# igashov/DiffLinker

Hardware: AMD Instinct MI355X
Metric: molecules/sec (500-step sample_chain) (higher is better)
Workload: dtype f32 (f16x3 split MFMA, fp32 accumulate)

## Files before the change

difflinker_amd/csrc/egnn_fc.hip:

```cpp
#include <hip/hip_runtime.h>
#include <stdint.h>
#include <stdlib.h>
#include <string.h>
#include <math.h>
#include <cmath>

#include <algorithm>
#include <atomic>
#include <vector>

#include "../../include/difflinker_hip.h"
#include "pack_layout.h"
#include "slot_order.h"


namespace {

constexpr int LDH = 132;
constexpr int NMAX = 55;
constexpr int NQMAX = 2 * NMAX;
constexpr int THREADS = 512;
constexpr int NWAVES = THREADS / 64;
constexpr int GWAVES = 8;
constexpr int GTHREADS = 64 * GWAVES;
constexpr int L_A = 0;
constexpr int L_B = L_A + NMAX * LDH;
constexpr int L_C = L_B + NMAX * LDH;
constexpr int L_W = L_C + NMAX * LDH;
constexpr int L_VEC = L_W + UNIT;
constexpr int L_XS = L_VEC + 4 * HID;
constexpr int L_X0 = L_XS + NQMAX * 4;
constexpr int L_Z = L_X0 + NQMAX * 4;
constexpr int L_LM = L_Z + NMAX * DMAX;
constexpr int L_FRAG = L_LM + 56;
constexpr int L_IDX = L_FRAG + 56;
constexpr int L_RCV = L_IDX + 112;
constexpr int L_RPOS = L_RCV + 56;
constexpr int L_MISC = L_RPOS + 56;
constexpr int MISC_WORDS = 40;
constexpr int L_FMAX = L_MISC + MISC_WORDS;
constexpr int L_DUMMY = L_FMAX + 8;
constexpr int L_PROG = L_DUMMY + LDH;
constexpr int L_TOTAL = L_PROG + 8;
constexpr int L_ZROW = L_XS + 4 * 56;
static_assert(L_ZROW + HID <= L_X0 && 56 >= NMAX + 1 && (L_ZROW % 4) == 0, "the zero row sits in the team-only part of the coordinate rows");
constexpr size_t LDS_BYTES = size_t(L_TOTAL) * 4;
static_assert(LDS_BYTES <= 163840, "LDS layout exceeds 160 KiB");
static_assert((L_B % 4) == 0 && (L_C % 4) == 0 && (L_W % 4) == 0 && (L_VEC % 4) == 0 && (L_XS % 4) == 0 &&
              (L_X0 % 4) == 0 && (L_Z % 4) == 0 && (L_DUMMY % 4) == 0, "16-byte alignment");
constexpr int L_TRIP3 = L_A + 2 * ST_CHUNK;
constexpr int L_AGGX3 = L_TRIP3 + 4 * 256;
static_assert(L_AGGX3 + 4 * (NMAX + 1) <= L_W && (L_TRIP3 % 4) == 0, "version-3 coordinate scratch must fit the h region behind the ring");

constexpr int TM_EPOCH = 2;
constexpr int TM_FAIL = 3;
constexpr int TM_ROWS = 4;
constexpr int TM_FLAGS = 6;
constexpr int TM_S = 8, TM_RANK = 9, TM_NOWN = 10;
constexpr int MS_NRCV = 12;
constexpr int MS_FULL = 13;
constexpr int CX_V3 = 38;

struct Lds {
    float *A, *B, *C, *W, *vec, *xs, *x0, *aggx, *z, *lm, *frag;
    int *idx, *rcv, *rpos, *misc;
    unsigned* fmax;
    float* dummy;
    int w;
};

__device__ __forceinline__ Lds lds_view(float* base) {
    Lds v;
    v.w = __builtin_amdgcn_readfirstlane(int(threadIdx.x) >> 6);
    v.A = base + L_A; v.B = base + L_B; v.C = base + L_C; v.W = base + L_W; v.vec = base + L_VEC;
    v.xs = base + L_XS; v.x0 = base + L_X0; v.z = base + L_Z;
    v.aggx = base + L_B;
    v.lm = base + L_LM; v.frag = base + L_FRAG;
    v.idx = reinterpret_cast<int*>(base + L_IDX); v.misc = reinterpret_cast<int*>(base + L_MISC);
    v.rcv = reinterpret_cast<int*>(base + L_RCV); v.rpos = reinterpret_cast<int*>(base + L_RPOS);
    v.fmax = reinterpret_cast<unsigned*>(base + L_FMAX);
    v.dummy = base + L_DUMMY;
    return v;
}

constexpr int PROF_MAX_EVENTS = 1024;
struct Prof {
    unsigned long long* buf;
    int n;
};
__device__ __forceinline__ void prof_event(Prof& pf, int w, int lane, int tag) {
#ifdef DL_PROFILE
    if (pf.buf != nullptr) {
        if (lane == 0 && pf.n < PROF_MAX_EVENTS) {
            unsigned long long* e = pf.buf + (size_t(w) * PROF_MAX_EVENTS + pf.n) * 2;
            e[0] = (unsigned long long)tag;
            e[1] = __builtin_amdgcn_s_memtime();
        }
        pf.n++;
    }
#else
    (void)pf; (void)w; (void)lane; (void)tag;
#endif
}

__device__ __forceinline__ void fine_event(Prof& pf, int w, int lane, int tag) {
// ... 68 lines not shown
    q.tid = 64 * q.w + q.lane;
    asm volatile("" : "+v"(q.tid));
    q.c = q.lane & 31; q.hh = q.lane >> 5;
    q.nt = q.w & 3; q.mt = q.w >> 2;
    return q;
}
struct NextPass {
    const float* base;
    bool equiv;
};
__device__ __forceinline__ void stage_next(const Lds& v, const NextPass& nx, int w, int tid) {
    if (nx.base == nullptr) return;
    stage_dma(v, nx.base + (nx.equiv ? E_W6T : G_W2T), nx.base + (nx.equiv ? E_VEC : G_VEC) + HID,
              nx.base + (nx.equiv ? E_VEC + 4 * HID : G_VEC + 6 * HID), w, tid);
}

__device__ __forceinline__ void store_row(const Lds& v, float* buf, int row, int nb, int col, float val) {
    float* p = (row < nb) ? buf + row * LDH + col : v.dummy + col;
    *p = val;
}

constexpr int FM_H0 = 0, FM_H1 = 1, FM_HG = 2, FM_AGG = 3, FM_XOWN = 4, FM_X2 = 5, FM_X02 = 6;

template <bool TEAM>
__device__ __forceinline__ float geo_scale(const Lds& v, const float* __restrict__ sc) {
    const float x2 = __uint_as_float(v.fmax[FM_X2]), x02 = __uint_as_float(v.fmax[FM_X02]);
    return fminf(scale_for(4.0f * x2) * scale_for(sc[6]), scale_for(4.0f * x02) * scale_for(sc[7]));
}

static_assert(SLOT_WAVES == GWAVES, "slot_order.h plans for the workgroup's waves");
constexpr int PB_STRIDE = LDH;
static_assert(NSLOT * PB_STRIDE <= L_W + UNIT, "partial-sum buffer must fit the P, Q, H, W2' regions");

#ifdef DL_TEST_HOOKS
__device__ int g_slots_receiver_major = 0;
#endif

__device__ __forceinline__ void split8t(const float (&u)[8], uint4& hi, uint4& lo) {
    unsigned h[4], l[4];
#pragma unroll
    for (int q = 0; q < 4; ++q) {
        const float a = u[2 * q], b = u[2 * q + 1];
        const float ah = __uint_as_float(__float_as_uint(a) & 0xffffe000u), bh = __uint_as_float(__float_as_uint(b) & 0xffffe000u);
        h[q] = __builtin_bit_cast(unsigned, __builtin_amdgcn_cvt_pkrtz(ah, bh));
        l[q] = __builtin_bit_cast(unsigned, __builtin_amdgcn_cvt_pkrtz(a - ah, b - bh));
    }
    hi = make_uint4(h[0], h[1], h[2], h[3]);
    lo = make_uint4(l[0], l[1], l[2], l[3]);
}

template <bool EQUIV, int PREC, bool ATT, bool TEAM>
__device__ __forceinline__ void pair_phase(const Lds& v, int nb, int w, int lane, const int8_t* __restrict__ emask, int N,
                                           float norm_constant, float sa, float inv_scale, const float* __restrict__ sc,
                                           float head, Prof& pf) {
    const int c = lane & 31, hh = lane >> 5;
    const int nrec = EQUIV ? v.misc[MS_NRCV] : (TEAM ? v.misc[TM_NOWN] : nb);
    const int S = TEAM ? v.misc[TM_S] : 1, rank = TEAM ? v.misc[TM_RANK] : 0;
#ifdef DL_TEST_HOOKS
    const SlotOrder so = slot_order(nrec, nb, g_slots_receiver_major != 0);
#else
    const SlotOrder so = slot_order(nrec, nb);
#endif
    const SlotLane sl = slot_lane(so, nb, 32 * w + c);
    const int q = so.q;
    const int nt = slot_wave_steps(so, w);
    const bool slot_ok = sl.ok;
    const int il = sl.il;
    const int li = EQUIV ? (slot_ok ? v.rcv[il] : 0) : il;
    const int i = rank + li * S;
    const int j0 = sl.j0;
    const int jn = sl.jn;
    const bool wave_active = nt > 0;

    floatx16 agg[4];
    float ax = 0.0f, ay = 0.0f, az = 0.0f;
#pragma unroll
    for (int mt = 0; mt < 4; ++mt) agg[mt] = splat16(0.0f);

    if (wave_active) {
        const float4 xi = *reinterpret_cast<const float4*>(v.xs + 4 * i);
        const float4 yi = *reinterpret_cast<const float4*>(v.x0 + 4 * i);
        const int8_t* mrow = emask ? emask + v.idx[i] * N : nullptr;
        const float* Pp_ = v.A + li * LDH + 4 * hh;
        const float* bias_p_ = v.vec + 2 * HID + 4 * hh;
        const float* w7_p_ = v.vec + 3 * HID + 4 * hh;
        float isa_s[8];
#pragma unroll
        for (int s_ = 0; s_ < 8; ++s_)
            isa_s[s_] = (PREC == 0) ? 1.0f
                : __int_as_float(__builtin_amdgcn_readfirstlane(__float_as_int(inv_pow2(sa * cload(sc, (EQUIV ? ES_NE : GS_NE) + s_)))));

        float ga[4];
        uint4 gaf[4];
        float sX = 1.0f, invS1 = 1.0f;
        if constexpr (PREC == 0) {
#pragma unroll
            for (int mt = 0; mt < 4; ++mt) ga[mt] = v.vec[(hh ? HID : 0) + 32 * mt + c];
        } else {
            const float s_wr = scale_for(sc[6]), s_wd = scale_for(sc[7]);
            const float S1 = geo_scale<TEAM>(v, sc);
            invS1 = inv_pow2(S1);
            sX = S1 * inv_pow2(hh ? s_wd : s_wr);
            const float s_w = hh ? s_wd : s_wr;
#pragma unroll
            for (int mt = 0; mt < 4; ++mt) {
                const float wv = v.vec[(hh ? HID : 0) + 32 * mt + c] * s_w;
                const float wh = __uint_as_float(__float_as_uint(wv) & 0xffffe000u);
// ... 241 lines not shown
                            __builtin_amdgcn_sched_barrier(0);
                        }
                    }
                } else
#pragma unroll
                for (int s = 0; s < 8; ++s) {
#pragma unroll
                    for (int i = 0; i < 12; ++i) {
                        const int m6 = i % 6, ge = 4 * (s + 1) + i / 3, ph = i % 3;
                        if (m6 == 0) {
                            const int ng = 2 * s + i / 6 + 1;
                            if (ng < 16) load_a(ng >> 1, ng & 1);
                        }
                        mfma_i(s, i);
                        if (i < 4 && s < 6 && !(s & 1)) load_qc((s + 2) >> 1, i);
                        if (i == 10 && s < 6 && !(s & 1)) g1 = mfma_h(gaf[(s + 2) >> 1], xf, Qc);
                        if (s < 7) {
                            if (ph == 0) { if ((ge & 1) == 0 && (ge >> 1) + 1 < 16) load_pq((ge >> 1) + 1); chunk_a(ge); }
                            if (ph == 1) chunk_b(ge);
                            if (ph == 2) chunk_c(ge);
                        }
                        __builtin_amdgcn_sched_barrier(0);
                    }
                }
                loop_event(pf, w, lane, 52);
                const float m = ok ? float(m_raw) : 0.0f;
                TileVecs tv[2];
                tv[0] = load_vecs(0);
#pragma unroll
                for (int mt = 0; mt < 4; ++mt) {
                    keep_vecs(tv[mt & 1]);
                    if (mt < 3) tv[(mt + 1) & 1] = load_vecs(mt + 1);
                    __builtin_amdgcn_sched_barrier(0);
                    epilogue(c2[mt], mt, tv[mt & 1], m);
                }
                if (ATT) attend(c2, m);
                loop_event(pf, w, lane, 53);
            }
            if (EQUIV) {
                float lo, hi;
                both_halves(ssum, lo, hi);
                float s_all = lo + hi;
                if (head != 0.0f)
                    s_all = head * (1.0f - 2.0f * __builtin_amdgcn_rcpf(1.0f + __builtin_amdgcn_exp2f(2.8853900817779268f * s_all)));
                const float den = sqrtf(r + 1e-8f) + norm_constant;
                const float f = ok ? s_all * float(m_raw) : 0.0f;
                ax += (dx / den) * f; ay += (dy / den) * f; az += (dz / den) * f;
            }
        }
        if (nt < q && lane == 0) prog[w] = q;
    }
    __builtin_amdgcn_s_setprio(0);
    prof_event(pf, w, lane, EQUIV ? 121 : 120);
    lds_barrier();
    if (lane == 0) reinterpret_cast<int*>(v.A - L_A + L_PROG)[w] = 0;
    int slot_w = 32 * w + c;
    asm volatile("" : "+v"(slot_w));
    const SlotLane sw = slot_lane(so, nb, slot_w);
    const int prow = sw.il * so.g + sw.c;
    float* pb = v.A + prow * PB_STRIDE;
    if (sw.ok) {
        if (!EQUIV) {
#pragma unroll
            for (int mt = 0; mt < 4; ++mt)
#pragma unroll
                for (int qq = 0; qq < 4; ++qq)
                    *reinterpret_cast<float4*>(pb + 32 * mt + 8 * qq + 4 * hh) =
                        make_float4(agg[mt][4 * qq], agg[mt][4 * qq + 1], agg[mt][4 * qq + 2], agg[mt][4 * qq + 3]);
        } else if (hh == 0) {
            *reinterpret_cast<float4*>(v.A + (v.misc[CX_V3] != 0 ? L_TRIP3 - L_A : 0) + 4 * prow) = make_float4(ax, ay, az, 0.0f);
        }
    }
}

struct AggRegs {
    float4 v[4];
};
__device__ __forceinline__ float pair_reduce_gcl(const Lds& v, int nown, int nb, int tid, AggRegs& out, float scale) {
    const SlotPlan pl = slot_plan(nown, nb);
    float am = 0.0f;
    const float* src[4];
    float4 s[4];
#pragma unroll
    for (int k = 0; k < 4; ++k) {
        const int e = tid + THREADS * k;
        src[k] = v.A + max(min(e >> 5, nown - 1), 0) * pl.g * PB_STRIDE + 4 * (e & 31);
        s[k] = make_float4(0.f, 0.f, 0.f, 0.f);
    }
    int ch = 0;
    for (; ch + 4 <= pl.g; ch += 4) {
        float4 p[4][4];
#pragma unroll
        for (int u = 0; u < 4; ++u)
#pragma unroll
            for (int k = 0; k < 4; ++k) p[u][k] = *reinterpret_cast<const float4*>(src[k] + (ch + u) * PB_STRIDE);
#pragma unroll
        for (int u = 0; u < 4; ++u)
#pragma unroll
            for (int k = 0; k < 4; ++k) { s[k].x += p[u][k].x; s[k].y += p[u][k].y; s[k].z += p[u][k].z; s[k].w += p[u][k].w; }
    }
    for (; ch < pl.g; ++ch) {
        float4 p[4];
#pragma unroll
        for (int k = 0; k < 4; ++k) p[k] = *reinterpret_cast<const float4*>(src[k] + ch * PB_STRIDE);
#pragma unroll
        for (int k = 0; k < 4; ++k) { s[k].x += p[k].x; s[k].y += p[k].y; s[k].z += p[k].z; s[k].w += p[k].w; }
// ... 556 lines not shown
    const int S = TEAM ? ctx_i(v, TM_S) : 1, rank = TEAM ? ctx_i(v, TM_RANK) : 0;
    float* hs = cx.hs;
    const NextPass nx = cx.nx;
    const LaneIds q = lane_ids(v);
    const int tid = q.tid, w = q.w, lane = q.lane;
    PreW2 pw;
    load_pre2(pw, nx, w, lane, nown);
    __builtin_amdgcn_sched_barrier(0);
    lds_barrier();
    const float xscale = (cx.flags & 4) ? 1.0f / float(N) : ((cx.flags & 2) ? ctx_f(v, CX_INVNORM) : 1.0f);
    pair_reduce_equiv<false>(v, nown, nb, tid, xscale);
    if (TEAM && tid == 0) v.fmax[FM_XOWN] = 0u;
    lds_barrier();
    stage_next(v, nx, w, tid);
    if constexpr (TEAM) {
        if (nb > NMAX && nx.base != nullptr)
            for (int e = tid; e < nown * 32; e += THREADS)
                *reinterpret_cast<float4*>(v.C + (e >> 5) * LDH + 4 * (e & 31)) = *reinterpret_cast<const float4*>(hs + HS_HF + (e >> 5) * HID + 4 * (e & 31));
    } else {
        if (tid == 0) v.fmax[FM_X2] = 0u;
        lds_barrier();
    }
    float n2 = 0.0f;
    if (tid < nown) {
        const float lm = v.lm[tid];
        const int a = rank + tid * S;
        const bool moves = v.rpos[tid] >= 0;
#pragma unroll
        for (int k = 0; k < 3; ++k) {
            float xn = v.xs[4 * a + k];
            if (moves) {
                xn += v.aggx[4 * tid + k] * lm;
                v.xs[4 * a + k] = xn;
            }
            n2 = fmaf(xn, xn, n2);
        }
    }
    block_max(&v.fmax[TEAM ? FM_XOWN : FM_X2], n2, lane);
    prof_event(pf, w, lane, 34);
    lds_barrier();
    prof_event(pf, w, lane, 10);
    open_pass<PREC, TEAM>(v, nb, nown, nx, hs, pf, pw, cx.pass + 1, cx.par);
}


typedef float floatx4 __attribute__((ext_vector_type(4)));
__device__ __forceinline__ floatx4 mfma16(const uint4& a, const uint4& b, floatx4 c) {
    return __builtin_amdgcn_mfma_f32_16x16x32_f16(__builtin_bit_cast(half8, a), __builtin_bit_cast(half8, b), c, 0, 0, 0);
}
constexpr int ST_AWAVES = 4;
constexpr int ST_PIECES = ST_CHUNK / 256 / 4;
__host__ __device__ constexpr int st_slot_off(int slot) { return slot < 2 ? L_W + slot * ST_CHUNK : L_A + (slot - 2) * ST_CHUNK; }
static_assert(L_A + 2 * ST_CHUNK <= L_W && 2 * ST_CHUNK == UNIT, "ring slots 2, 3 must fit below the W2' region");
__host__ __device__ constexpr int st_slot(int c, int nc) { return (c + ((4 - nc) & 3)) & 3; }

struct BOp {
    uint4 hi[4], lo[4];
};
__device__ __forceinline__ float4* st_tile(float* tiles, int w, int ot, int lane) {
    return reinterpret_cast<float4*>(tiles) + (w * 8 + ot) * 64 + lane;
}
__device__ __forceinline__ void st_load_rows(BOp& b, const float* rows, int l, int kg, float s) {
    const float* rp = rows + l * LDH + 4 * kg;
#pragma unroll
    for (int sl = 0; sl < 4; ++sl) {
        const float4 a = *reinterpret_cast<const float4*>(rp + 32 * sl), c4 = *reinterpret_cast<const float4*>(rp + 32 * sl + 16);
        const float u[8] = {a.x * s, a.y * s, a.z * s, a.w * s, c4.x * s, c4.y * s, c4.z * s, c4.w * s};
        split8t(u, b.hi[sl], b.lo[sl]);
    }
}
template <int SLOT>
__device__ __forceinline__ void st_mma_chunk(const float* lds0, const BOp& b, floatx4 (&acc)[4], int lane) {
    const uint4* Wc = reinterpret_cast<const uint4*>(lds0 + st_slot_off(SLOT)) + lane;
#pragma unroll
    for (int t = 0; t < 4; ++t) acc[t] = floatx4{0.f, 0.f, 0.f, 0.f};
#pragma unroll
    for (int sl = 0; sl < 4; ++sl) {
        uint4 ah[4], al[4];
#ifdef DL_KO_DSR
#pragma unroll
        for (int t = 0; t < 4; ++t) { ah[t] = b.hi[(sl + t) & 3]; al[t] = b.lo[(sl + t) & 3]; }
#else
#pragma unroll
        for (int t = 0; t < 4; ++t) { ah[t] = Wc[((t * 4 + sl) * 2 + 0) * 64]; al[t] = Wc[((t * 4 + sl) * 2 + 1) * 64]; }
#endif
#ifdef DL_KO_MFMA
#pragma unroll
        for (int t = 0; t < 4; ++t) { acc[t][0] += __uint_as_float(al[t].x ^ ah[t].y); acc[t][1] += __uint_as_float(al[t].z ^ ah[t].w); }
#else
#pragma unroll
        for (int t = 0; t < 4; ++t) acc[t] = mfma16(al[t], b.hi[sl], acc[t]);
#pragma unroll
        for (int t = 0; t < 4; ++t) acc[t] = mfma16(ah[t], b.lo[sl], acc[t]);
#pragma unroll
        for (int t = 0; t < 4; ++t) acc[t] = mfma16(ah[t], b.hi[sl], acc[t]);
#endif
    }
}
template <int SLOT>
__device__ __forceinline__ void st_issue(float* lds0, const float* __restrict__ src, int hw, int lane) {
    typedef const __attribute__((address_space(1))) void* gptr_t;
    typedef __attribute__((address_space(3))) void* lptr_t;
    const float4* s4 = reinterpret_cast<const float4*>(src) + lane;
#ifdef DL_KO_DMA
    (void)s4; (void)lds0; (void)hw;
#else
#pragma unroll
    for (int it = 0; it < ST_PIECES; ++it) {
        const int piece = it * 4 + hw;
        __builtin_amdgcn_global_load_lds((gptr_t)(s4 + piece * 64), (lptr_t)(lds0 + st_slot_off(SLOT) + piece * 256), 16, 0, 0);
    }
#endif
}
template <int HALF>
__device__ __forceinline__ void st_issue_image(const Lds& v, const NextPass& nx, int hw, int lane) {
    typedef const __attribute__((address_space(1))) void* gptr_t;
    typedef __attribute__((address_space(3))) void* lptr_t;
    const float* wimg = nx.base + (nx.equiv ? E_W6T : G_W2T);
    const float* vecs = nx.base + (nx.equiv ? E_VEC : G_VEC) + HID;
    const float* vec4 = nx.base + (nx.equiv ? E_VEC + 4 * HID : G_VEC + 6 * HID);
    if (HALF == 1 && hw < 2) {
        const int t2 = 64 * hw + lane;
        const float4* src = (t2 < 96) ? reinterpret_cast<const float4*>(vecs) + t2 : reinterpret_cast<const float4*>(vec4) + (t2 - 96);
        __builtin_amdgcn_global_load_lds((gptr_t)src, (lptr_t)(v.vec + 256 * hw), 16, 0, 0);
    }
    const float4* s4 = reinterpret_cast<const float4*>(wimg) + lane;
#pragma unroll
    for (int it = 0; it < ST_PIECES; ++it) {
        const int piece = HALF * 32 + it * 4 + hw;
        __builtin_amdgcn_global_load_lds((gptr_t)(s4 + piece * 64), (lptr_t)(v.W + piece * 256), 16, 0, 0);
    }
}
template <int N>
__device__ __forceinline__ void st_wait_vm() {
    if constexpr (N <= 0) asm volatile("s_waitcnt vmcnt(0)" ::: "memory");
    else asm volatile("s_waitcnt vmcnt(%0)" :: "n"(N) : "memory");
}
template <int V>
struct IC { static constexpr int value = V; };

template <bool TEAM, bool POST, bool NEXT_EQ>
__device__ __forceinline__ void stream_phase(const Lds& v, Prof& pf, const AggRegs* ar) {
    constexpr int NC = (POST ? 6 : 0) + 4;
    constexpr int C_P = POST ? 6 : 0;
    const PassCtx cx = pass_ctx(v);
    const LaneIds q = lane_ids(v);
    const int tid = q.tid, w = q.w, lane = q.lane;
    const int nb = cx.nb;
    const int nown = TEAM ? ctx_i(v, TM_NOWN) : nb;
    float* hs = cx.hs;
    const int pass_open = cx.pass + 1;
    const float* wp = ctx_p<const float>(v, CX_WP);
    const int sub = ctx_i(v, CX_SUB);
    const float* g = POST ? cx.g : nullptr;
    const float* nxb = pass_weights(wp, pass_open, sub);
    const NextPass nx = {nxb, NEXT_EQ};
    const float* sc = POST ? g + G_SCALE : nullptr;
    const float* scn = nxb + (NEXT_EQ ? E_SCALE : G_SCALE);
    const float* vecn = nxb + (NEXT_EQ ? E_VEC : G_VEC);
    float* lds0 = v.A - L_A;
    const bool loader = w >= ST_AWAVES;
    const int hw = w - ST_AWAVES, wa = w;
    const int n = lane & 15, kg = lane >> 4;
    const int ta = wa;
    const int l = 16 * ta + n;
    const bool awave = !loader && 16 * ta < nown;
    const bool valid = awave && l < nown;
    const int lc = max(min(l, nown - 1), 0);
    auto chunk_src = [&](int c) -> const float* {
        if (POST && c < C_P) return g + G_ST_POST + c * ST_CHUNK;
        return nxb + (NEXT_EQ ? E_ST_PRE : G_ST_PRE) + (c - C_P) * ST_CHUNK;
    };
    float4 hold[8];
    if (awave) {
#pragma unroll
        for (int ot = 0; ot < 8; ++ot) hold[ot] = *st_tile(hs + HS_HT, ta, ot, lane);
    }
    const int par = cx.par;
    float hmax = 0.f, aggmax = 0.f, s_agg = 1.f, s_t = 1.f, s_hn = 1.f, inv2 = 1.f;
    if constexpr (POST) {
        hmax = __uint_as_float(v.fmax[FM_H0 + par]);
        aggmax = __uint_as_float(v.fmax[FM_AGG]);
        s_agg = scale_for(aggmax);
        const float y3b = cload(sc, SC_L1_W3A) * hmax + cload(sc, SC_L1_W3B) * aggmax + cload(sc, SC_B3);
        s_t = scale_for(y3b);
        const float hnb = hmax + cload(sc, SC_L1_W4) * y3b + cload(sc, SC_B4);
        s_hn = scale_for(hnb);
        if (tid == 0 && (beyond_f16_range(aggmax) || beyond_f16_range(y3b) || beyond_f16_range(hnb))) atomicOr(&v.misc[1], NAN_RANGE | 3);
        inv2 = inv_pow2(s_t * cload(sc, 4));
    }
    const float s_h0 = scale_for(__uint_as_float(v.fmax[FM_H0 + par]));
    const float s_hf = POST ? s_hn : s_h0;
    constexpr int AGG_OFF = st_slot_off(st_slot(3, NC));
    if constexpr (POST) {
#pragma unroll
        for (int k = 0; k < 4; ++k) {
            const int e = tid + THREADS * k;
            if (e < nown * 32) *reinterpret_cast<float4*>(lds0 + AGG_OFF + (e >> 5) * LDH + 4 * (e & 31)) = ar->v[k];
        }
    }
    if (loader) {
        st_issue<st_slot(0, NC)>(lds0, chunk_src(0), hw, lane);
        prof_event(pf, w, lane, 200);
        auto lstep = [&](auto C_) {
            constexpr int C = decltype(C_)::value;
            constexpr int behind = (C >= 1 && C + 1 < NC ? ST_PIECES : 0) + (C == NC - 2 ? ST_PIECES : 0) + (C == NC - 1 ? 2 * ST_PIECES : 0);
            st_wait_vm<behind>();
            fine_event(pf, w, lane, 220 + C);
            lds_barrier();
            fine_event(pf, w, lane, 210 + C);
            if constexpr (C == 0) {
                st_issue<st_slot(1, NC)>(lds0, chunk_src(1), hw, lane);
                st_issue<st_slot(2, NC)>(lds0, chunk_src(2), hw, lane);
            }
            if constexpr (C == 1) st_wait_vm<ST_PIECES>();
            if constexpr (C >= 1 && C + 2 < NC) st_issue<st_slot(C + 2, NC)>(lds0, chunk_src(C + 2), hw, lane);
            if constexpr (C == NC - 3) st_issue_image<0>(v, nx, hw, lane);
            if constexpr (C == NC - 2) st_issue_image<1>(v, nx, hw, lane);
        };
        lstep(IC<0>{}); lstep(IC<1>{}); lstep(IC<2>{}); lstep(IC<3>{});
        if constexpr (NC > 4) { lstep(IC<4>{}); lstep(IC<5>{}); }
        if constexpr (NC > 6) { lstep(IC<6>{}); lstep(IC<7>{}); }
        if constexpr (NC > 8) { lstep(IC<8>{}); lstep(IC<9>{}); }
        fine_event(pf, w, lane, 240);
        lds_barrier();
        prof_event(pf, w, lane, 250);
    } else {
    BOp bh, bagg, bout, bin;
    floatx4 acc[4];
    float4 t0p[4];
    float4 res2[8], bb4[8];
    float4 Pout[8], Qout[8];
    float hm = 0.f;
    float S1 = 1.f;
    if (!TEAM) {
        const float x2 = __uint_as_float(v.fmax[FM_X2]), x02 = __uint_as_float(v.fmax[FM_X02]);
        S1 = fminf(scale_for(4.0f * x2) * scale_for(cload(scn, 6)), scale_for(4.0f * x02) * scale_for(cload(scn, 7)));
    }
    const float live = valid ? 1.0f : 0.0f;
    if (awave) {
        const float sb = s_h0 * live;
#pragma unroll
        for (int sl = 0; sl < 4; ++sl) {
            const float4 a = hold[2 * sl], c4 = hold[2 * sl + 1];
            const float u[8] = {a.x * sb, a.y * sb, a.z * sb, a.w * sb, c4.x * sb, c4.y * sb, c4.z * sb, c4.w * sb};
            split8t(u, bh.hi[sl], bh.lo[sl]);
        }
    }
    prof_event(pf, w, lane, 200);
    auto step = [&](auto C_) {
        constexpr int C = decltype(C_)::value;
        fine_event(pf, w, lane, 230 + C);
        lds_barrier();
        fine_event(pf, w, lane, 210 + C);
        if (!awave) return;
        constexpr bool IS_T0 = POST && C < 4 && (C & 1) == 0, IS_MLP1 = POST && C < 4 && (C & 1) == 1, IS_MLP2 = POST && (C == 4 || C == 5);
        constexpr bool IS_P = C >= C_P && C < C_P + 2;
        constexpr int half = (POST && C < 4) ? (C >> 1) : (C & 1);
        float4 bias[4];
        if constexpr (IS_P || IS_T0) {
#pragma unroll
            for (int t = 0; t < 4; ++t)
                bias[t] = *reinterpret_cast<const float4*>((IS_T0 ? g + G_VEC + 4 * HID : vecn) + 16 * (4 * half + t) + 4 * kg);
        }
        if constexpr (POST && C == 3) {
#pragma unroll
            for (int ot = 0; ot < 8; ++ot) {
                res2[ot] = *st_tile(hs + HS_HT, ta, ot, lane);
                bb4[ot] = *reinterpret_cast<const float4*>(g + G_VEC + 5 * HID + 16 * ot + 4 * kg);
            }
        }
        if constexpr (POST && C == 0) st_load_rows(bagg, lds0 + AGG_OFF, lc, kg, s_agg * live);
        if constexpr (IS_T0) st_mma_chunk<st_slot(C, NC)>(lds0, bh, acc, lane);
        else if constexpr (IS_MLP1) st_mma_chunk<st_slot(C, NC)>(lds0, bagg, acc, lane);
        else if constexpr (IS_MLP2) st_mma_chunk<st_slot(C, NC)>(lds0, bin, acc, lane);
        else st_mma_chunk<st_slot(C, NC)>(lds0, POST ? bin : bh, acc, lane);
        float4 res[4];
#pragma unroll
        for (int t = 0; t < 4; ++t) {
            const int ot = 4 * half + t, nt = ot >> 1;
            if constexpr (IS_T0) {
                const float inv = inv_pow2(s_h0 * cload(sc, GS_SW_W3A + nt));
                const float4 b3 = bias[t];
                t0p[t] = make_float4(fmaf(acc[t][0], inv, b3.x), fmaf(acc[t][1], inv, b3.y), fmaf(acc[t][2], inv, b3.z), fmaf(acc[t][3], inv, b3.w));
            } else if constexpr (IS_MLP1) {
                const float inv = inv_pow2(s_agg * cload(sc, GS_SW_W3B + nt)), stn = s_t * cload(sc, GS_NT + nt) * live;
                const float4 t0 = t0p[t];
                res[t] = make_float4(silu_u(fmaf(acc[t][0], inv, t0.x)) * stn, silu_u(fmaf(acc[t][1], inv, t0.y)) * stn,
                                     silu_u(fmaf(acc[t][2], inv, t0.z)) * stn, silu_u(fmaf(acc[t][3], inv, t0.w)) * stn);
            } else if constexpr (IS_MLP2) {
                const float4 hd = res2[ot], b4 = bb4[ot];
                const float4 hv = make_float4(fmaf(acc[t][0], inv2, hd.x + b4.x), fmaf(acc[t][1], inv2, hd.y + b4.y),
                                              fmaf(acc[t][2], inv2, hd.z + b4.z), fmaf(acc[t][3], inv2, hd.w + b4.w));
                *st_tile(hs + HS_HT, ta, ot, lane) = hv;
                if (valid) hm = fmaxf(fmaxf(hm, fmaxf(fabsf(hv.x), fabsf(hv.y))), fmaxf(fabsf(hv.z), fabsf(hv.w)));
                const float shl = s_hn * live;
                res[t] = make_float4(hv.x * shl, hv.y * shl, hv.z * shl, hv.w * shl);
            } else if constexpr (IS_P) {
                const float inv = inv_pow2(s_hf * cload(scn, (NEXT_EQ ? ES_SW_W5A : GS_SW_W1A) + nt));
                const float4 b1 = bias[t];
                Pout[ot] = make_float4(fmaf(acc[t][0], inv, b1.x), fmaf(acc[t][1], inv, b1.y), fmaf(acc[t][2], inv, b1.z), fmaf(acc[t][3], inv, b1.w));
            } else {
                const float inv = inv_pow2(s_hf * cload(scn, (NEXT_EQ ? ES_SW_W5A : GS_SW_W1A) + 4 + nt)) * S1;
                Qout[ot] = make_float4(acc[t][0] * inv, acc[t][1] * inv, acc[t][2] * inv, acc[t][3] * inv);
            }
        }
        if constexpr (IS_MLP1 || IS_MLP2) {
#pragma unroll
            for (int sp = 0; sp < 2; ++sp) {
                const float4 a = res[2 * sp], c4 = res[2 * sp + 1];
                const float u[8] = {a.x, a.y, a.z, a.w, c4.x, c4.y, c4.z, c4.w};
                split8t(u, bout.hi[2 * half + sp], bout.lo[2 * half + sp]);
            }
            if constexpr (half == 1) bin = bout;
            if constexpr (C == 5) block_max(&v.fmax[FM_H0 + (par ^ 1)], hm, lane);
        }
    };
    step(IC<0>{}); step(IC<1>{}); step(IC<2>{}); step(IC<3>{});
    if constexpr (NC > 4) { step(IC<4>{}); step(IC<5>{}); }
    if constexpr (NC > 6) { step(IC<6>{}); step(IC<7>{}); }
    if constexpr (NC > 8) { step(IC<8>{}); step(IC<9>{}); }
    fine_event(pf, w, lane, 240);
    lds_barrier();
    prof_event(pf, w, lane, 250);
    if (valid) {
#pragma unroll
        for (int ot = 0; ot < 8; ++ot) {
            *reinterpret_cast<float4*>(v.A + l * LDH + 16 * ot + 4 * kg) = Pout[ot];
            *reinterpret_cast<float4*>(v.B + l * LDH + 16 * ot + 4 * kg) = Qout[ot];
        }
    }
    }
    if (tid == 0) {
        if constexpr (POST) { v.fmax[FS_HS] = __float_as_uint(s_hn); v.misc[CX_PAR] = par ^ 1; }
        v.misc[CX_PASS] = pass_open;
    }
    if constexpr (TEAM) {
        prof_event(pf, w, lane, 110);
        lds_barrier();
        team_exchange_q<1>(v, nb, tid, scn, pass_open == 0, POST ? (par ^ 1) : par, pf);
    }
    prof_event(pf, w, lane, 11);
    dma_wait();
    lds_barrier();
}


template <int PREC, bool TEAM, bool ATT>
__device__ __forceinline__ void gcl_pass3(const Lds& v, Prof& pf) {
    {
    const PassCtx cx = pass_ctx(v);
    const int nb = cx.nb, N = cx.N, par = cx.par;
    const int8_t* emask = cx.em;
    const float* sc = cx.g + G_SCALE;
    const LaneIds q = lane_ids(v);
    const int tid = q.tid, w = q.w, lane = q.lane;
    prof_event(pf, w, lane, 12);
    if (tid == 0) { v.fmax[FM_H0 + (par ^ 1)] = 0u; v.fmax[FM_AGG] = 0u; }
    const float hmax = __uint_as_float(v.fmax[TEAM ? FM_HG : FM_H0 + par]);
    const float x2 = __uint_as_float(v.fmax[FM_X2]), x02 = __uint_as_float(v.fmax[FM_X02]);
    const float pqb = (cload(sc, SC_L1_W1A) + cload(sc, SC_L1_W1B)) * hmax + cload(sc, SC_B1);
    const float u1b = pqb + 4.0f * (x2 * cload(sc, GS_WRW) + x02 * cload(sc, GS_WDW));
    const float sa = scale_for(u1b);
    const float accs = sa * cload(sc, 5);
    if (tid == 0 && (beyond_f16_range(u1b) || beyond_f16_range(hmax) || beyond_f16_range(4.0f * x2) || beyond_f16_range(4.0f * x02)))
        atomicOr(&v.misc[1], NAN_RANGE | 3);
    if constexpr (ATT) pair_phase<false, PREC, true, TEAM>(v, nb, w, lane, emask, N, 0.0f, sa, inv_pow2(accs), sc, cload(sc, 8), pf);
    else pair_phase<false, PREC, false, TEAM>(v, nb, w, lane, emask, N, 0.0f, sa, inv_pow2(accs), sc, 0.0f, pf);
    prof_event(pf, w, lane, 13);
    }
    AggRegs ar;
    bool next_eq;
    {
        const PassCtx cx = pass_ctx(v);
        const int nown = TEAM ? ctx_i(v, TM_NOWN) : cx.nb;
        const LaneIds q = lane_ids(v);
        next_eq = cx.nx.equiv;
        lds_barrier();
        prof_event(pf, q.w, q.lane, 20);
        const float am = pair_reduce_gcl(v, nown, cx.nb, q.tid, ar, (cx.flags & 4) ? 1.0f / float(cx.N) : 1.0f);
        block_max(&v.fmax[FM_AGG], am, q.lane);
        prof_event(pf, q.w, q.lane, 21);
        lds_barrier();
        prof_event(pf, q.w, q.lane, 22);
    }
    if (next_eq) stream_phase<TEAM, true, true>(v, pf, &ar);
    else stream_phase<TEAM, true, false>(v, pf, &ar);
}

template <int PREC, bool TEAM>
__device__ __forceinline__ void equiv_pass3(const Lds& v, Prof& pf) {
    {
    const PassCtx cx = pass_ctx(v);
    const int nb = cx.nb, N = cx.N, par = cx.par;
    const int8_t* emask = cx.em;
    const float* sc = cx.g + E_SCALE;
    const float norm_constant = ctx_f(v, CX_NORMC);
    const LaneIds q = lane_ids(v);
    const int w = q.w, lane = q.lane;
    prof_event(pf, w, lane, 32);
    const float hmax = __uint_as_float(v.fmax[TEAM ? FM_HG : FM_H0 + par]);
    const float x2 = __uint_as_float(v.fmax[FM_X2]), x02 = __uint_as_float(v.fmax[FM_X02]);
    const float pqb = (cload(sc, SCE_L1_W5A) + cload(sc, SCE_L1_W5B)) * hmax + cload(sc, SCE_B5);
    const float u1b = pqb + 4.0f * (x2 * cload(sc, ES_WRW) + x02 * cload(sc, ES_WDW));
    const float sa = scale_for(u1b);
    const float accs = sa * cload(sc, 2);
    if (q.tid == 0 && (beyond_f16_range(u1b) || beyond_f16_range(hmax) || beyond_f16_range(4.0f * x2) || beyond_f16_range(4.0f * x02)))
        atomicOr(&v.misc[1], NAN_RANGE | 3);
    const float phi = cload(sc, ES_W7L1) * fmaf(cload(sc, ES_L1_W6), u1b, cload(sc, ES_B6));
    const bool proven = 2.0f * float(nb) * phi < 1e37f;
    if (!proven) {
        const bool widen = ctx_i(v, MS_FULL) == 0;
        __syncthreads();
        if (widen) {
            const int tid_ = q.tid;
            receivers_all(v, TEAM ? ctx_i(v, TM_NOWN) : nb, tid_);
            __syncthreads();
        }
    }
    pair_phase<true, PREC, false, TEAM>(v, nb, w, lane, emask, N, norm_constant, sa, inv_pow2(accs), sc,
                                        (cx.flags & 2) ? ctx_f(v, CX_CRANGE) : 0.0f, pf);
    prof_event(pf, w, lane, 33);
    }
    const PassCtx cx = pass_ctx(v);
    const int nb = cx.nb, N = cx.N;
    const int nown = TEAM ? ctx_i(v, TM_NOWN) : nb;
    const int S = TEAM ? ctx_i(v, TM_S) : 1, rank = TEAM ? ctx_i(v, TM_RANK) : 0;
    const bool more = cx.nx.base != nullptr;
    const LaneIds q = lane_ids(v);
    const int tid = q.tid, lane = q.lane;
    lds_barrier();
    const float xscale = (cx.flags & 4) ? 1.0f / float(N) : ((cx.flags & 2) ? ctx_f(v, CX_INVNORM) : 1.0f);
    pair_reduce_equiv<true>(v, nown, nb, tid, xscale);
    if (tid == 0) v.fmax[TEAM ? FM_XOWN : FM_X2] = 0u;
    lds_barrier();
    const float* aggx = v.A - L_A + L_AGGX3;
    float n2 = 0.0f;
// ... 39 lines not shown
    if (tid < 8) reinterpret_cast<int*>(v.A - L_A + L_PROG)[tid] = 0;
    if (!TEAM && tid < HID) (v.A - L_A + L_ZROW)[tid] = 0.0f;
    prof_event(pf, w, lane, 1);
    {
        if (tid < 8) v.fmax[tid] = 0u;
        __syncthreads();
    }
    const NextPass first = {wp + OFF_BLOCKS, false};
    if (!v3) stage_next(v, first, w, tid);
    if (tid < 4 * nown) {
        const int l = tid >> 2, k = tid & 3, a = rank + l * S;
        const float xv = (k < 3) ? v.z[l * DMAX + k] : 0.0f;
        v.xs[4 * a + k] = xv;
        v.x0[4 * a + k] = xv;
    }
    {
        float n2 = 0.0f;
        if (tid < nown) {
            const float x0 = v.z[tid * DMAX], x1 = v.z[tid * DMAX + 1], x2 = v.z[tid * DMAX + 2];
            n2 = x0 * x0 + x1 * x1 + x2 * x2;
        }
        const unsigned b = wave_max_u32(__float_as_uint(n2));
        if (lane == 0) {
            if (TEAM) lds_max_u32(&v.fmax[FM_XOWN], b);
            else { lds_max_u32(&v.fmax[FM_X2], b); lds_max_u32(&v.fmax[FM_X02], b); }
        }
    }
    {
        const int f = tid & (HID - 1);
        float wrow[FINP];
        const float4* wsrc = reinterpret_cast<const float4*>(wp + OFF_EMB_W + f * FINP);
#pragma unroll
        for (int q = 0; q < FINP / 4; ++q) {
            const float4 t4 = wsrc[q];
            wrow[4 * q] = t4.x; wrow[4 * q + 1] = t4.y; wrow[4 * q + 2] = t4.z; wrow[4 * q + 3] = t4.w;
        }
        const float be = wp[OFF_EMB_B + f];
        const float* ctxp = ctx_p<const float>(v, CX_CTXP);
        const int ct = ctx_i(v, CX_CT);
        const int nctx = fin - nf - ct;
        float hmax = 0.0f;
        for (int l = tid >> 7; l < nown; l += THREADS / HID) {
            const int pos = v.idx[rank + l * S];
            float acc = be;
#pragma unroll
            for (int k = 0; k < FINP; ++k) {
                float hin = 0.0f;
                if (k < nf) hin = v.z[l * DMAX + 3 + k];
                else if (k < nf + ct) hin = tfeat;
                else if (k < fin) hin = ctxp[pos * nctx + (k - nf - ct)];
                acc = fmaf(wrow[k], hin, acc);
            }
            if (v3) {
                hs[HS_HT + ((((l >> 4) * 8 + (f >> 4)) * 64 + 16 * ((f >> 2) & 3) + (l & 15)) * 4) + (f & 3)] = acc;
            } else {
            v.B[l * LDH + f] = acc;
            {
                const int r = l & 31;
                hs[HS_HT + ((((l >> 5) * 4 + (f >> 5)) * 4 + (r >> 3)) * 64 + (f & 31) + 32 * ((r >> 2) & 1)) * 4 + (r & 3)] = acc;
            }
            }
            hmax = fmaxf(hmax, fabsf(acc));
        }
        block_max(&v.fmax[FM_H0], hmax, lane);
    }
    __syncthreads();
    if (v3) {
        if constexpr (PREC != 0 && !TEAM) {
        if (tid == 0 && beyond_f16_range(__uint_as_float(v.fmax[FM_H0]))) atomicOr(&v.misc[1], NAN_RANGE | 3);
        prof_event(pf, w, lane, 2);
        stream_phase<TEAM, false, false>(v, pf, nullptr);
        const int sub = ctx_i(v, CX_SUB);
#pragma nounroll
        for (int p = 0; p < npass; p += sub + 1) {
#pragma nounroll
            for (int gi = 0; gi < sub; ++gi) gcl_pass3<PREC, TEAM, ATT>(v, pf);
            equiv_pass3<PREC, TEAM>(v, pf);
        }
        prof_event(pf, w, lane, 3);
        __syncthreads();
        head_phase<TEAM>(v, true);
        }
    } else {
    {
        const float s0 = (PREC != 0) ? scale_for(__uint_as_float(v.fmax[FM_H0])) : 1.0f;
        for (int e = tid; e < nown * 32; e += THREADS)
            put_quad<PREC>(v.C + (e >> 5) * LDH, 4 * (e & 31), *reinterpret_cast<const float4*>(v.B + (e >> 5) * LDH + 4 * (e & 31)), s0);
        if (PREC != 0 && tid == 0) {
            v.fmax[FS_HS] = __float_as_uint(s0);
            if (beyond_f16_range(__uint_as_float(v.fmax[FM_H0]))) atomicOr(&v.misc[1], NAN_RANGE | 3);
        }
    }
    __syncthreads();
    prof_event(pf, w, lane, 2);
    {
        PreW2 pw;
        load_pre2(pw, first, w, lane, nown);
        open_pass<PREC, TEAM>(v, nb, nown, first, hs, pf, pw, 0, 0);
    }
    const int sub = ctx_i(v, CX_SUB);
#pragma nounroll
    for (int p = 0; p < npass; p += sub + 1) {
#pragma nounroll
        for (int gi = 0; gi < sub; ++gi) gcl_pass2<PREC, TEAM, ATT>(v, pf);
        equiv_pass2<PREC, TEAM>(v, pf);
    }
    prof_event(pf, w, lane, 3);
    __syncthreads();
    head_phase<TEAM>(v, false);
    }
    prof_event(pf, w, lane, 4);
}

template <bool TEAM>
__device__ __forceinline__ void head_phase(const Lds& v, bool v3) {
    const int tid = lane_ids(v).tid;
    const int nb = ctx_i(v, 0), nf = ctx_i(v, CX_NF);
    const int nown = TEAM ? ctx_i(v, TM_NOWN) : nb;
    const int S = TEAM ? ctx_i(v, TM_S) : 1, rank = TEAM ? ctx_i(v, TM_RANK) : 0;
    const float* wp = ctx_p<const float>(v, CX_WP);
    const float* hs = ctx_p<const float>(v, CX_HS);
    float* eps = v.A;
    int nanbits = 0;
    for (int e = tid; e < nown * nf; e += THREADS) {
        const int a = e / nf, o = e - a * nf;
        const int r = a & 31;
        const float* wo = wp + OFF_OUT_W + o * HID;
        float acc = wp[OFF_OUT_B + o];
        if (v3) {
            const float* hp = hs + HS_HT + ((a >> 4) * 8 * 64 + (a & 15)) * 4;
#pragma unroll
            for (int ot = 0; ot < 8; ++ot)
#pragma unroll
                for (int kg = 0; kg < 4; ++kg) {
                    const float4 hv = *reinterpret_cast<const float4*>(hp + (ot * 64 + 16 * kg) * 4);
                    const float4 wv = *reinterpret_cast<const float4*>(wo + 16 * ot + 4 * kg);
                    acc = fmaf(hv.x, wv.x, acc); acc = fmaf(hv.y, wv.y, acc);
                    acc = fmaf(hv.z, wv.z, acc); acc = fmaf(hv.w, wv.w, acc);
                }
        } else {
        const float* hp = hs + HS_HO + ((a >> 5) * 4 * 16 + (r & 3) + 4 * (r >> 3)) * 64 + 32 * ((r >> 2) & 1);
#pragma unroll
        for (int nt4 = 0; nt4 < 4; ++nt4)
#pragma unroll 8
            for (int q = 0; q < 8; ++q) {
                const float4 hv = *reinterpret_cast<const float4*>(hp + nt4 * 16 * 64 + 4 * q);
                const float4 wv = *reinterpret_cast<const float4*>(wo + 32 * nt4 + 4 * q);
                acc = fmaf(hv.x, wv.x, acc); acc = fmaf(hv.y, wv.y, acc);
                acc = fmaf(hv.z, wv.z, acc); acc = fmaf(hv.w, wv.w, acc);
            }
        }
        (void)r;
        eps[a * DMAX + 3 + o] = acc;
        if (acc != acc) nanbits |= 2;
    }
    if (tid < 4 * nown && (tid & 3) < 3) {
        const int l = tid >> 2, a = rank + l * S;
        const float vel = v.xs[4 * a + (tid & 3)] - v.x0[4 * a + (tid & 3)];
        eps[l * DMAX + (tid & 3)] = vel;
        if (vel != vel) nanbits |= 1;
    }
    if (TEAM && tid == 0 && v.misc[TM_FAIL] != 0) nanbits |= 8;
    if (nanbits) atomicOr(&v.misc[1], nanbits);
    __syncthreads();
}

__device__ __forceinline__ void build_receivers(const Lds& v, int nown, int tid) {
    if (tid < 64) {
        const bool rec = tid < nown && v.lm[tid] != 0.0f;
        const unsigned long long bal = __ballot(rec);
        const int pos = __popcll(bal & ((1ull << tid) - 1ull));
        if (rec) v.rcv[pos] = tid;
        if (tid < NMAX + 1) v.rpos[tid] = rec ? pos : -1;
        if (tid == 0) { v.misc[MS_NRCV] = __popcll(bal); v.misc[MS_FULL] = (__popcll(bal) == nown) ? 1 : 0; }
    }
}

__device__ __forceinline__ int compact_atoms(const Lds& v, const int8_t* __restrict__ node_mask_b, int N, int tid) {
    if (tid < 64) {
        int count = 0;
        for (int base = 0; base < N; base += 64) {
            const int a = base + tid;
            const bool real = (a < N) && (node_mask_b[a] != 0);
            const unsigned long long bal = __ballot(real);
            const int pos = count + __popcll(bal & ((1ull << tid) - 1ull));
            if (real && pos < NQMAX) v.idx[pos] = a;
            count += __popcll(bal);
        }
// ... 1282 lines not shown
```

Baseline: 584.6.

## Keep version-3 node features resident in LDS region C instead of global scratch

Moves the v3 node-feature rows (HS_HT) from a global scratch buffer into LDS region C, laid out row-major with the LDH stride. The embedding, the stream phase's residual loads and stores, and the output head now read and write LDS instead of global memory. To make room, the ring slot order is changed so the aggregate rows and coordinate scratch fit below C. Feature data that the pair phase and ring slot 3 would overwrite is parked in registers or VGPR keeps and restored after barriers. This removes global-memory round trips per pass, at the cost of extra barriers, higher register pressure and fragile aliasing of the LDS regions.

```diff
diff --git a/difflinker_amd/csrc/egnn_fc.hip b/difflinker_amd/csrc/egnn_fc.hip
--- a/difflinker_amd/csrc/egnn_fc.hip
+++ b/difflinker_amd/csrc/egnn_fc.hip
@@ -48,9 +48,15 @@
 static_assert(LDS_BYTES <= 163840, "LDS layout exceeds 160 KiB");
 static_assert((L_B % 4) == 0 && (L_C % 4) == 0 && (L_W % 4) == 0 && (L_VEC % 4) == 0 && (L_XS % 4) == 0 &&
               (L_X0 % 4) == 0 && (L_Z % 4) == 0 && (L_DUMMY % 4) == 0, "16-byte alignment");
-constexpr int L_TRIP3 = L_A + 2 * ST_CHUNK;
+constexpr int L_TRIP3 = L_A + ST_CHUNK;
 constexpr int L_AGGX3 = L_TRIP3 + 4 * 256;
-static_assert(L_AGGX3 + 4 * (NMAX + 1) <= L_W && (L_TRIP3 % 4) == 0, "version-3 coordinate scratch must fit the h region behind the ring");
+static_assert(L_AGGX3 + 4 * (NMAX + 1) <= L_C && (L_TRIP3 % 4) == 0, "version-3 coordinate scratch must stay below the node features");
+constexpr int C_QUADS = NMAX * LDH / 4;
+static_assert(C_QUADS <= 4 * THREADS && (NMAX * LDH) % 4 == 0, "four float4 per thread park region C");
+typedef float quad_t __attribute__((ext_vector_type(4)));
+struct ParkRegs {
+    quad_t a, b, c, d;
+};
 
 constexpr int TM_EPOCH = 2;
 constexpr int TM_FAIL = 3;
@@ -225,7 +231,7 @@
 template <bool EQUIV, int PREC, bool ATT, bool TEAM>
 __device__ __forceinline__ void pair_phase(const Lds& v, int nb, int w, int lane, const int8_t* __restrict__ emask, int N,
                                            float norm_constant, float sa, float inv_scale, const float* __restrict__ sc,
-                                           float head, Prof& pf) {
+                                           float head, Prof& pf, ParkRegs* park = nullptr) {
     const int c = lane & 31, hh = lane >> 5;
     const int nrec = EQUIV ? v.misc[MS_NRCV] : (TEAM ? v.misc[TM_NOWN] : nb);
     const int S = TEAM ? v.misc[TM_S] : 1, rank = TEAM ? v.misc[TM_RANK] : 0;
@@ -573,6 +579,15 @@
     }
     __builtin_amdgcn_s_setprio(0);
     prof_event(pf, w, lane, EQUIV ? 121 : 120);
+    if (!EQUIV && park != nullptr) {
+        int t3 = 64 * w + lane;
+        asm volatile("" : "+v"(t3));
+        const quad_t* cq = reinterpret_cast<const quad_t*>(v.C);
+        park->a = cq[min(t3, C_QUADS - 1)];
+        park->b = cq[min(t3 + THREADS, C_QUADS - 1)];
+        park->c = cq[min(t3 + 2 * THREADS, C_QUADS - 1)];
+        park->d = cq[min(t3 + 3 * THREADS, C_QUADS - 1)];
+    }
     lds_barrier();
     if (lane == 0) reinterpret_cast<int*>(v.A - L_A + L_PROG)[w] = 0;
     int slot_w = 32 * w + c;
@@ -1235,14 +1250,15 @@
 constexpr int ST_PIECES = ST_CHUNK / 256 / 4;
 __host__ __device__ constexpr int st_slot_off(int slot) { return slot < 2 ? L_W + slot * ST_CHUNK : L_A + (slot - 2) * ST_CHUNK; }
 static_assert(L_A + 2 * ST_CHUNK <= L_W && 2 * ST_CHUNK == UNIT, "ring slots 2, 3 must fit below the W2' region");
-__host__ __device__ constexpr int st_slot(int c, int nc) { return (c + ((4 - nc) & 3)) & 3; }
+__host__ __device__ constexpr int st_slot(int c, int nc) { return c == nc - 1 ? 3 : (c + (3 - (nc - 2) % 3 + 2) % 3) % 3; }
+static_assert(st_slot(8, 10) == 2 && st_slot(9, 10) == 3 && st_slot(7, 10) == 1 && st_slot(6, 10) == 0 && st_slot(0, 10) == 0 &&
+              st_slot(2, 4) == 2 && st_slot(3, 4) == 3 && st_slot(1, 4) == 1 && st_slot(0, 4) == 0, "ring order");
+constexpr int ST_KEEP = L_A + 2 * ST_CHUNK - L_C;
+static_assert(ST_KEEP > 0 && ST_KEEP % 4 == 0 && ST_KEEP / 4 <= 2 * 256, "two float4 per loader thread keep the feature rows under slot 3");
 
 struct BOp {
     uint4 hi[4], lo[4];
 };
-__device__ __forceinline__ float4* st_tile(float* tiles, int w, int ot, int lane) {
-    return reinterpret_cast<float4*>(tiles) + (w * 8 + ot) * 64 + lane;
-}
 __device__ __forceinline__ void st_load_rows(BOp& b, const float* rows, int l, int kg, float s) {
     const float* rp = rows + l * LDH + 4 * kg;
 #pragma unroll
@@ -1331,7 +1347,6 @@
     const int tid = q.tid, w = q.w, lane = q.lane;
     const int nb = cx.nb;
     const int nown = TEAM ? ctx_i(v, TM_NOWN) : nb;
-    float* hs = cx.hs;
     const int pass_open = cx.pass + 1;
     const float* wp = ctx_p<const float>(v, CX_WP);
     const int sub = ctx_i(v, CX_SUB);
@@ -1354,11 +1369,7 @@
         if (POST && c < C_P) return g + G_ST_POST + c * ST_CHUNK;
         return nxb + (NEXT_EQ ? E_ST_PRE : G_ST_PRE) + (c - C_P) * ST_CHUNK;
     };
-    float4 hold[8];
-    if (awave) {
-#pragma unroll
-        for (int ot = 0; ot < 8; ++ot) hold[ot] = *st_tile(hs + HS_HT, ta, ot, lane);
-    }
+    float* hrow = v.C + lc * LDH + 4 * kg;
     const int par = cx.par;
     float hmax = 0.f, aggmax = 0.f, s_agg = 1.f, s_t = 1.f, s_hn = 1.f, inv2 = 1.f;
     if constexpr (POST) {
@@ -1374,7 +1385,8 @@
     }
     const float s_h0 = scale_for(__uint_as_float(v.fmax[FM_H0 + par]));
     const float s_hf = POST ? s_hn : s_h0;
-    constexpr int AGG_OFF = st_slot_off(st_slot(3, NC));
+    constexpr int AGG_OFF = st_slot_off(st_slot(2, NC));
+    static_assert(!POST || (st_slot(2, NC) != st_slot(0, NC) && st_slot_off(st_slot(2, NC)) + NMAX * LDH <= L_C), "aggregate rows: clear of chunk 0 and of the node features");
     if constexpr (POST) {
 #pragma unroll
         for (int k = 0; k < 4; ++k) {
@@ -1383,8 +1395,13 @@
         }
     }
     if (loader) {
+        if constexpr (POST) lds_barrier();
         st_issue<st_slot(0, NC)>(lds0, chunk_src(0), hw, lane);
         prof_event(pf, w, lane, 200);
+        floatx4 keep0 = {0.f, 0.f, 0.f, 0.f}, keep1 = keep0;
+        const int kq = 64 * hw + lane;
+        const unsigned keep_addr = (unsigned)(uintptr_t)(__attribute__((address_space(3))) float*)(v.C + 4 * kq);
+        constexpr int KEEP1 = ST_KEEP / 4 - 256;
         auto lstep = [&](auto C_) {
             constexpr int C = decltype(C_)::value;
             constexpr int behind = (C >= 1 && C + 1 < NC ? ST_PIECES : 0) + (C == NC - 2 ? ST_PIECES : 0) + (C == NC - 1 ? 2 * ST_PIECES : 0);
@@ -1397,6 +1414,11 @@
                 st_issue<st_slot(2, NC)>(lds0, chunk_src(2), hw, lane);
             }
             if constexpr (C == 1) st_wait_vm<ST_PIECES>();
+            if constexpr (C == NC - 3) {
+                static_assert(st_slot(C + 2, NC) == 3 && (!POST || C > 5), "slot 3: the last chunk only, after the features' last store");
+                asm volatile("ds_read_b128 %0, %2\n\tds_read_b128 %1, %2 offset:4096\n\ts_waitcnt lgkmcnt(0)"
+                             : "=&v"(keep0), "=&v"(keep1) : "v"(keep_addr) : "memory");
+            }
             if constexpr (C >= 1 && C + 2 < NC) st_issue<st_slot(C + 2, NC)>(lds0, chunk_src(C + 2), hw, lane);
             if constexpr (C == NC - 3) st_issue_image<0>(v, nx, hw, lane);
             if constexpr (C == NC - 2) st_issue_image<1>(v, nx, hw, lane);
@@ -1408,6 +1430,8 @@
         fine_event(pf, w, lane, 240);
         lds_barrier();
         prof_event(pf, w, lane, 250);
+        asm volatile("ds_write_b128 %0, %1" :: "v"(keep_addr), "v"(keep0) : "memory");
+        if (kq < KEEP1) asm volatile("ds_write_b128 %0, %1 offset:4096" :: "v"(keep_addr), "v"(keep1) : "memory");
     } else {
     BOp bh, bagg, bout, bin;
     floatx4 acc[4];
@@ -1421,14 +1445,16 @@
         S1 = fminf(scale_for(4.0f * x2) * scale_for(cload(scn, 6)), scale_for(4.0f * x02) * scale_for(cload(scn, 7)));
     }
     const float live = valid ? 1.0f : 0.0f;
+    if constexpr (POST) lds_barrier();
     if (awave) {
         const float sb = s_h0 * live;
 #pragma unroll
         for (int sl = 0; sl < 4; ++sl) {
-            const float4 a = hold[2 * sl], c4 = hold[2 * sl + 1];
+            const float4 a = *reinterpret_cast<const float4*>(hrow + 32 * sl), c4 = *reinterpret_cast<const float4*>(hrow + 32 * sl + 16);
             const float u[8] = {a.x * sb, a.y * sb, a.z * sb, a.w * sb, c4.x * sb, c4.y * sb, c4.z * sb, c4.w * sb};
             split8t(u, bh.hi[sl], bh.lo[sl]);
         }
+        if constexpr (POST) st_load_rows(bagg, lds0 + AGG_OFF, lc, kg, s_agg * live);
     }
     prof_event(pf, w, lane, 200);
     auto step = [&](auto C_) {
@@ -1449,11 +1475,10 @@
         if constexpr (POST && C == 3) {
 #pragma unroll
             for (int ot = 0; ot < 8; ++ot) {
-                res2[ot] = *st_tile(hs + HS_HT, ta, ot, lane);
+                res2[ot] = *reinterpret_cast<const float4*>(hrow + 16 * ot);
                 bb4[ot] = *reinterpret_cast<const float4*>(g + G_VEC + 5 * HID + 16 * ot + 4 * kg);
             }
         }
-        if constexpr (POST && C == 0) st_load_rows(bagg, lds0 + AGG_OFF, lc, kg, s_agg * live);
         if constexpr (IS_T0) st_mma_chunk<st_slot(C, NC)>(lds0, bh, acc, lane);
         else if constexpr (IS_MLP1) st_mma_chunk<st_slot(C, NC)>(lds0, bagg, acc, lane);
         else if constexpr (IS_MLP2) st_mma_chunk<st_slot(C, NC)>(lds0, bin, acc, lane);
@@ -1475,7 +1500,7 @@
                 const float4 hd = res2[ot], b4 = bb4[ot];
                 const float4 hv = make_float4(fmaf(acc[t][0], inv2, hd.x + b4.x), fmaf(acc[t][1], inv2, hd.y + b4.y),
                                               fmaf(acc[t][2], inv2, hd.z + b4.z), fmaf(acc[t][3], inv2, hd.w + b4.w));
-                *st_tile(hs + HS_HT, ta, ot, lane) = hv;
+                if (valid) *reinterpret_cast<float4*>(hrow + 16 * ot) = hv;
                 if (valid) hm = fmaxf(fmaxf(hm, fmaxf(fabsf(hv.x), fabsf(hv.y))), fmaxf(fabsf(hv.z), fabsf(hv.w)));
                 const float shl = s_hn * live;
                 res[t] = make_float4(hv.x * shl, hv.y * shl, hv.z * shl, hv.w * shl);
@@ -1531,6 +1556,7 @@
 
 template <int PREC, bool TEAM, bool ATT>
 __device__ __forceinline__ void gcl_pass3(const Lds& v, Prof& pf) {
+    ParkRegs park;
     {
     const PassCtx cx = pass_ctx(v);
     const int nb = cx.nb, N = cx.N, par = cx.par;
@@ -1548,8 +1574,8 @@
     const float accs = sa * cload(sc, 5);
     if (tid == 0 && (beyond_f16_range(u1b) || beyond_f16_range(hmax) || beyond_f16_range(4.0f * x2) || beyond_f16_range(4.0f * x02)))
         atomicOr(&v.misc[1], NAN_RANGE | 3);
-    if constexpr (ATT) pair_phase<false, PREC, true, TEAM>(v, nb, w, lane, emask, N, 0.0f, sa, inv_pow2(accs), sc, cload(sc, 8), pf);
-    else pair_phase<false, PREC, false, TEAM>(v, nb, w, lane, emask, N, 0.0f, sa, inv_pow2(accs), sc, 0.0f, pf);
+    if constexpr (ATT) pair_phase<false, PREC, true, TEAM>(v, nb, w, lane, emask, N, 0.0f, sa, inv_pow2(accs), sc, cload(sc, 8), pf, &park);
+    else pair_phase<false, PREC, false, TEAM>(v, nb, w, lane, emask, N, 0.0f, sa, inv_pow2(accs), sc, 0.0f, pf, &park);
     prof_event(pf, w, lane, 13);
     }
     AggRegs ar;
@@ -1566,6 +1592,10 @@
         prof_event(pf, q.w, q.lane, 21);
         lds_barrier();
         prof_event(pf, q.w, q.lane, 22);
+        quad_t* cq = reinterpret_cast<quad_t*>(v.C) + q.tid;
+        cq[0] = park.a; cq[THREADS] = park.b; cq[2 * THREADS] = park.c;
+        if (q.tid + 3 * THREADS < C_QUADS) cq[3 * THREADS] = park.d;
+        static_assert(3 * THREADS <= C_QUADS, "the first three rounds are whole");
     }
     if (next_eq) stream_phase<TEAM, true, true>(v, pf, &ar);
     else stream_phase<TEAM, true, false>(v, pf, &ar);
@@ -1711,7 +1741,7 @@
                 acc = fmaf(wrow[k], hin, acc);
             }
             if (v3) {
-                hs[HS_HT + ((((l >> 4) * 8 + (f >> 4)) * 64 + 16 * ((f >> 2) & 3) + (l & 15)) * 4) + (f & 3)] = acc;
+                v.C[l * LDH + f] = acc;
             } else {
             v.B[l * LDH + f] = acc;
             {
@@ -1787,12 +1817,12 @@
         const float* wo = wp + OFF_OUT_W + o * HID;
         float acc = wp[OFF_OUT_B + o];
         if (v3) {
-            const float* hp = hs + HS_HT + ((a >> 4) * 8 * 64 + (a & 15)) * 4;
+            const float* hp = v.C + a * LDH;
 #pragma unroll
             for (int ot = 0; ot < 8; ++ot)
 #pragma unroll
                 for (int kg = 0; kg < 4; ++kg) {
-                    const float4 hv = *reinterpret_cast<const float4*>(hp + (ot * 64 + 16 * kg) * 4);
+                    const float4 hv = *reinterpret_cast<const float4*>(hp + 16 * ot + 4 * kg);
                     const float4 wv = *reinterpret_cast<const float4*>(wo + 16 * ot + 4 * kg);
                     acc = fmaf(hv.x, wv.x, acc); acc = fmaf(hv.y, wv.y, acc);
                     acc = fmaf(hv.z, wv.z, acc); acc = fmaf(hv.w, wv.w, acc);
```

Result: no change. 587.1 (median of 6 runs) (+0.4%).
